# Critical-Infrastructure-Systems-Lab/ldsr

Hardware: AMD Instinct MI355X
Metric: restart x EM-iteration / s (T=1000, p=1, q=2) (higher is better)
Workload: dtype f64; 1 GPU; cfg2: synthetic T=1000 p=1 q=2, 1 series x 4096 restarts/GPU, niter=100, tol=0, dense mask; cells_rank0=4096, cells_total=4096, niter=100, algo=3

## Files before the change

ldsr_amd/csrc/em_pair_impl.h:

```cpp
#pragma once
#include "em_scan_impl.h"

__host__ __device__ constexpr long pair_image_doubles(int L, int PP, int QQ, int LPC = 32) {
    return img_doubles(L, LPC, PP, QQ);
}
__host__ __device__ constexpr long pair_strip_doubles(int L) { return (long)64 * (L - 1); }

__host__ __device__ constexpr long pair_tri_doubles(int PP, int QQ, int LPC = 32) {
    return (long)LPC * 2 * scan_pairs(PP, QQ);
}
#ifndef LDSR_STEADY
#define LDSR_STEADY 1
#endif
#ifndef LDSR_STEADY_PF
#define LDSR_STEADY_PF 4
#endif
#ifndef LDSR_STEADY_PF2
#define LDSR_STEADY_PF2 6
#endif
#ifndef LDSR_LEAD_CLOSED_VAR
#define LDSR_LEAD_CLOSED_VAR 1
#endif
#ifndef LDSR_STEADY_SBMASK
#define LDSR_STEADY_SBMASK 0x6
#endif
#ifndef LDSR_STEADY_MIN_L
#define LDSR_STEADY_MIN_L 24
#endif
#ifndef LDSR_PAIR_SPF
#define LDSR_PAIR_SPF 1
#endif
#ifndef LDSR_QUAD_SPF_LONG
#define LDSR_QUAD_SPF_LONG 1
#endif
#ifndef LDSR_PAIR_SPF_MAXL
#define LDSR_PAIR_SPF_MAXL 23
#endif
__host__ __device__ constexpr bool pair_spf(int PP, int QQ, int L, int LPC = 32) {
    return LDSR_PAIR_SPF && PP + QQ <= 8 && (L <= LDSR_PAIR_SPF_MAXL || (LDSR_QUAD_SPF_LONG && LPC == 16 && PP + QQ <= 4));
}
__host__ __device__ constexpr int pair_steady_ntr(int L, int LPC) { return L - 1; }
__host__ __device__ constexpr bool pair_steady(int L, int LPC, int PP, int QQ) {
    if (!LDSR_STEADY) return false;
    return LPC == 32 && L >= LDSR_STEADY_MIN_L &&
           (pair_image_doubles(L, PP, QQ, LPC) + 8 * pair_strip_doubles(L) + pair_tri_doubles(PP, QQ, LPC)) * 8 <= 160 * 1024;
}

__host__ __device__ constexpr bool pair_wide(int PP, int QQ) { return PP > 4 || QQ > 4; }
__host__ __device__ constexpr bool pair_member_fits(int L, int LPC, int PP, int QQ) {
    return (pair_image_doubles(L, PP, QQ, LPC) + (pair_wide(PP, QQ) ? 4 : 8) * pair_strip_doubles(L)) * 8 <= 160 * 1024;
}
constexpr int kPairLeadMaxL = 16;
__host__ __device__ constexpr bool pair_variant(int PP, int QQ, int L, int LPC, bool queue, bool lead) {
    if (!pair_member_fits(L, LPC, PP, QQ) || (lead && L > kPairLeadMaxL)) return false;
    return pair_wide(PP, QQ) ? lead && queue : true;
}

__device__ __forceinline__ double shfl_d(double x, int src_lane) { return __shfl(x, src_lane, 64); }

template <int LPC>
__device__ __forceinline__ void rscan_cross(double &P, double &G, double &H, int lane) {
    if constexpr (LPC == 32) {
        const double G1 = readlane_d(G, 16), H1 = readlane_d(H, 16), P1 = readlane_d(P, 16);
        const double G3 = readlane_d(G, 48), H3 = readlane_d(H, 48), P3 = readlane_d(P, 48);
        const int row = lane >> 4;
        const double Gs = row == 0 ? G1 : row == 2 ? G3 : 0.0;
        const double Hs = row == 0 ? H1 : row == 2 ? H3 : 0.0;
        const double Ps = row == 0 ? P1 : row == 2 ? P3 : 1.0;
        G = fma(P, Gs, G);
        H = fma(P * P, Hs, H);
        P *= Ps;
    }
}

#ifndef LDSR_LEAD_PIPE
#define LDSR_LEAD_PIPE 1
#endif
#ifndef LDSR_LEAD_PIPE_MAXP
#define LDSR_LEAD_PIPE_MAXP 2
#endif
__host__ __device__ constexpr bool lead_pipe(int PP) { return LDSR_LEAD_PIPE && PP <= LDSR_LEAD_PIPE_MAXP; }
template <int PP, int LPC, typename F>
__device__ __forceinline__ void lead_walk(const double *lup, int nj, int nA, F &&step) {
    constexpr int G = PP >= 4 ? 1 : 4 / PP;
    constexpr long ROW = (long)LPC * PP;
    double ua[G][PP], ub[G][PP];
    auto rd = [&](const double *base, double (&w)[G][PP]) {
#pragma unroll
        for (int i = 0; i < G; i++)
#pragma unroll
            for (int p_ = 0; p_ < PP; p_++) w[i][p_] = base[i * ROW + p_];
    };
    auto rdc = [&](int j0, double (&w)[G][PP]) {
#pragma unroll
        for (int i = 0; i < G; i++) {
            const int jj = min(j0 + i, nA - 1);
#pragma unroll
            for (int p_ = 0; p_ < PP; p_++) w[i][p_] = lup[jj * ROW + p_];
        }
    };
    if (nj <= 0) return;
    int j0 = 0;
    rdc(0, ua);
    const double *base = lup;
    for (; j0 + 3 * G <= nj; j0 += 2 * G, base += 2 * G * ROW) {
        rd(base + G * ROW, ub);
#pragma unroll
        for (int i = 0; i < G; i++) step(j0 + i, ua[i]);
        rd(base + 2 * G * ROW, ua);
#pragma unroll
        for (int i = 0; i < G; i++) step(j0 + G + i, ub[i]);
    }
    double uc[G][PP];
    rdc(j0 + G, ub);
    rdc(j0 + 2 * G, uc);
#pragma unroll
    for (int i = 0; i < G; i++)
        if (j0 + i < nj) step(j0 + i, ua[i]);
#pragma unroll
    for (int i = 0; i < G; i++)
        if (j0 + G + i < nj) step(j0 + G + i, ub[i]);
#pragma unroll
    for (int i = 0; i < G; i++)
        if (j0 + 2 * G + i < nj) step(j0 + 2 * G + i, uc[i]);
}

template <int PP, int QQ>
struct PairSweepOut {
    double aSyx, aTx1x, aPall, aSxx, likq, lsp, tLv, X0v, V0v;
    double aSxv[QQ], aTx1u[PP], aTux[PP];
    int sneg;
};

template <int PP, int QQ, int L, int LPC, bool DENSE>
__device__ __forceinline__ void pair_generic_sweeps(PairSweepOut<PP, QQ> &o, const Theta<PP, QQ> &th,
                                                    const double *ys, double *hs, unsigned obsmask,
                                                    int lane, int nl, int rp, double x_t1, double v_t1) {
    constexpr int KV = img_values(PP, QQ);
    const int vl = lane & (LPC - 1);
    auto val = [&](int j, int i) -> double { return ys[img_off(j, i, KV, LPC, L) + vl * 2]; };
    auto Yat = [&](int j) { return val(j, 0); };
    auto Uat = [&](int j, int k) { return val(j, 1 + k); };
    auto Vat = [&](int j, int k) { return val(j, 1 + PP + k); };
    constexpr bool SPF = pair_spf(PP, QQ, L, LPC) && (L <= LDSR_PAIR_SPF_MAXL || DENSE);
    constexpr int SPFD = scan_pairs(PP, QQ) <= 2 ? 2 : 1;
    constexpr int SPFN = SPFD + 1;
    constexpr int KH2 = 2 * (KV / 2);
    constexpr bool KODD = (KV & 1) != 0;
    struct StepRing {
        double w[SPFN][KH2 > 0 ? KH2 : 1];
        double o[2][2];
    };
    auto ring_rd = [&](double (&w)[KH2 > 0 ? KH2 : 1], double (&o)[2][2], int jn, bool with_odd) {
#pragma unroll
        for (int i = 0; i < KH2; i++) w[i] = val(jn, i);
        if (KODD && with_odd) {
            o[(jn >> 1) & 1][0] = val(jn & ~1, KV - 1);
            o[(jn >> 1) & 1][1] = val(jn | 1, KV - 1);
        }
    };
    const bool act = vl < nl, tail = vl < rp;
    const int lastLane = nl - 1;
    const double A = th.A, C = th.C, Q = th.Q, R = th.R;
    const double A2 = A * A, C2 = C * C;
    const double rR = fast_rcp(R);
    const double C2R = C2 * rR, ACR = A * C * rR, alpha = fma(Q, C2R, A2);
    auto e_at = [&](int j) {
        double e = Yat(j);
#pragma unroll
        for (int q_ = 0; q_ < QQ; q_++) e = fma(-th.D[q_], Vat(j, q_), e);
        return e;
    };
    auto bu_at = [&](int j) {
        double bu = 0.0;
#pragma unroll
        for (int p_ = 0; p_ < PP; p_++) bu = fma(th.B[p_], Uat(j, p_), bu);
        return bu;
    };
    auto e_of = [&](const double (&w)[KH2 > 0 ? KH2 : 1], const double (&o)[2][2], int j) {
        auto vv = [&](int i) { return i < KH2 ? w[i] : o[(j >> 1) & 1][j & 1]; };
        double e = vv(0);
#pragma unroll
        for (int q_ = 0; q_ < QQ; q_++) e = fma(-th.D[q_], vv(1 + PP + q_), e);
        return e;
    };
    auto bu_of = [&](const double (&w)[KH2 > 0 ? KH2 : 1], const double (&o)[2][2], int j) {
        auto vv = [&](int i) { return i < KH2 ? w[i] : o[(j >> 1) & 1][j & 1]; };
        double bu = 0.0;
#pragma unroll
        for (int p_ = 0; p_ < PP; p_++) bu = fma(th.B[p_], vv(1 + p_), bu);
        return bu;
    };
    double Jv[L], gv_[L];
    double hlast = 0.0;
    double likq = 0.0, lsp = 0.0, tLv = 0.0, X0v = 0.0, V0v = 0.0;
    int sneg = 0;
    double aSyx = 0.0, aTx1x = 0.0, aPall = 0.0, aSxx = 0.0;
    double aSxv[QQ], aTx1u[PP], aTux[PP];
#pragma unroll
    for (int q_ = 0; q_ < QQ; q_++) aSxv[q_] = 0.0;
#pragma unroll
    for (int p_ = 0; p_ < PP; p_++) { aTx1u[p_] = 0.0; aTux[p_] = 0.0; }

    PMat M;
    M.m00 = 1.0; M.m01 = 0.0; M.m10 = 0.0; M.m11 = 1.0; M.m20 = 0.0; M.m21 = 0.0; M.m22 = 1.0;
    if constexpr (DENSE) {
        const double mx = fmax(alpha, 1.0);
        const int ke = -__builtin_amdgcn_frexp_exp(mx);
        const double c = __builtin_amdgcn_ldexp(1.0, ke), cinv = __builtin_amdgcn_ldexp(1.0, -ke);
        const double al_ = alpha * c, Q_ = Q * c, C2R_ = C2R * c, A_ = A * c;
        double p00 = al_, p01 = Q_, p10 = C2R_, p11 = c;
        double q00 = 1.0, q01 = 0.0, q10 = 0.0, q11 = 1.0;
        bool have = false;
#pragma unroll
        for (int bit = 0; (1 << bit) <= L - 1; bit++) {
            if ((L - 1) & (1 << bit)) {
                if (!have) { q00 = p00; q01 = p01; q10 = p10; q11 = p11; have = true; }
                else {
                    const double t00 = fma(q00, p00, q01 * p10), t01 = fma(q00, p01, q01 * p11);
                    const double t10 = fma(q10, p00, q11 * p10), t11 = fma(q10, p01, q11 * p11);
// ... 23 lines not shown
                StepRing r;
#pragma unroll
                for (int d = 0; d < SPFD; d++)
                    if (L - 1 - d >= 0) ring_rd(r.w[(L - 1 - d) % SPFN], r.o, L - 1 - d, d == 0 || ((L - 1 - d) & 1) != 0);
                __builtin_amdgcn_sched_barrier(0x6);
#pragma unroll
                for (int j = L - 1; j >= 0; j--) {
                    if (j - SPFD >= 0) ring_rd(r.w[(j - SPFD) % SPFN], r.o, j - SPFD, ((j - SPFD) & 1) != 0);
                    if (j < L - 1 || tail) row_c(j, e_of(r.w[j % SPFN], r.o, j), bu_of(r.w[j % SPFN], r.o, j));
                    __builtin_amdgcn_sched_barrier(0x6);
                }
            } else {
                if (tail) row(L - 1);
#pragma unroll
                for (int j = L - 2; j >= 0; j--) row(j);
            }
            M.m00 = tail ? r00 : q00; M.m01 = tail ? r01 : q01;
            M.m10 = tail ? r10 : q10; M.m11 = tail ? r11 : q11;
            M.m20 = ra; M.m21 = rb; M.m22 = rcc * cinv;
            prenorm(M);
        }
    } else if (act) {
        auto f1c = [&](int j, double e, double bu) {
            const bool o = (obsmask >> j) & 1u;
            gv_[j] = e; Jv[j] = bu;
            const double a00 = o ? alpha : A2;
            const double g = o ? C2R : 0.0;
            const double s20 = o ? fma(bu, C2R, ACR * e) : 0.0;
            if (j == 0) {
                M.m00 = a00; M.m01 = Q; M.m10 = g; M.m11 = 1.0; M.m20 = s20; M.m21 = bu; M.m22 = A;
            } else {
                M = pstep(a00, Q, g, s20, bu, A, M);
            }
            if ((j & 15) == 15 && j < L - 2) prenorm(M);
        };
        auto f1 = [&](int j) { f1c(j, e_at(j), bu_at(j)); };
        if constexpr (SPF) {
            StepRing r;
#pragma unroll
            for (int d = 0; d < SPFD; d++)
                if (d <= L - 1) ring_rd(r.w[d % SPFN], r.o, d, (d & 1) == 0);
            __builtin_amdgcn_sched_barrier(0x6);
#pragma unroll
            for (int j = 0; j < L - 1; j++) {
                if (j + SPFD <= L - 1) ring_rd(r.w[(j + SPFD) % SPFN], r.o, j + SPFD, ((j + SPFD) & 1) == 0);
                f1c(j, e_of(r.w[j % SPFN], r.o, j), bu_of(r.w[j % SPFN], r.o, j));
                __builtin_amdgcn_sched_barrier(0x6);
            }
            if (tail) f1c(L - 1, e_of(r.w[(L - 1) % SPFN], r.o, L - 1), bu_of(r.w[(L - 1) % SPFN], r.o, L - 1));
        } else {
#pragma unroll
            for (int j = 0; j < L - 1; j++) f1(j);
            if (tail) f1(L - 1);
        }
        prenorm(M);
    }

    M = pmul(M, pdpp<DPP_ROW_SHR(1), 0xF>(M));
    M = pmul(M, pdpp<DPP_ROW_SHR(2), 0xF>(M));
    M = pmul(M, pdpp<DPP_ROW_SHR(4), 0xF>(M));
    prenorm(M);
    M = pmul(M, pdpp<DPP_ROW_SHR(8), 0xF>(M));
    if constexpr (LPC >= 32) M = pmul(M, pdpp<DPP_ROW_BCAST15, 0xA>(M));
    const double n_in = v_t1, d_in = 1.0, x_in = x_t1;
    double n_e = fma(M.m00, n_in, M.m01 * d_in);
    double d_e = fma(M.m10, n_in, M.m11 * d_in);
    double x_e = fma(M.m20, n_in, fma(M.m21, d_in, M.m22 * x_in));
    n_e = dppd<DPP_WAVE_SHR1, 0xF>(n_in, n_e);
    d_e = dppd<DPP_WAVE_SHR1, 0xF>(d_in, d_e);
    x_e = dppd<DPP_WAVE_SHR1, 0xF>(x_in, x_e);
    if (vl == 0) { n_e = n_in; d_e = d_in; x_e = x_in; }
    double Xp, Vp;
    {
        const double rd = fast_rcp(d_e);
        Vp = n_e * rd;
        Xp = x_e * rd;
    }

    double sprod = 1.0, Xu = 0.0, Vu = 0.0;
    int sexp = 0;
    double sg = fma(C2, Vp, R);
    double r0 = fast_rcp(sg);
    double Pi = 1.0, G = 0.0, H = 0.0;
    auto f2 = [&](int j) {
        const bool o = DENSE || ((obsmask >> j) & 1u);
        const double e = gv_[j], bu = Jv[j];
        const double r = o ? r0 : 0.0;
        const double sl = o ? sg : 1.0;
        sprod *= sl;
        sneg |= __double2hiint(sl);
        if ((j & 7) == 7) {
            sexp += __builtin_amdgcn_frexp_exp(sprod);
            sprod = __builtin_amdgcn_frexp_mant(sprod);
        }
        const double w = Vp * r;
        const double K = C * w;
        if (DENSE) Vu = R * w;
        else Vu = fma(-(C2 * w), Vp, Vp);
        const double dl = fma(-C, Xp, e);
        Xu = fma(K, dl, Xp);
        likq = fma(dl * r, dl, likq);
        const double Vp1 = fma(A2, Vu, Q);
        const double Xp1 = fma(A, Xu, bu);
        sg = fma(C2, Vp1, R);
        const double z = fast_rcp(sg * Vp1);
        const double rp1 = sg * z;
        r0 = Vp1 * z;
        const double AVu = A * Vu;
        double J = AVu * rp1;
        double g = fma(-J, Xp1, Xu);
        double h = fma(-J, AVu, Vu);
        if (j >= L - 2) {
            const bool fin = (vl == lastLane) && (j == (tail ? L - 1 : L - 2));
            J = fin ? 0.0 : J;
            g = fin ? Xu : g;
            h = fin ? Vu : h;
        }
        Jv[j] = J; gv_[j] = g;
        if (j < L - 1) hs[j * 64] = h; else hlast = h;
        G = fma(Pi, g, G);
        H = fma(Pi * Pi, h, H);
        Pi *= J;
        Xp = Xp1;
        Vp = Vp1;
        if ((j & 7) == 7) __builtin_amdgcn_sched_barrier(0);
    };
    if (act) {
#pragma unroll
        for (int j = 0; j < L - 1; j++) f2(j);
        if (tail) f2(L - 1);
    }
    tLv = fma(Xu, Xu, Vu);
    lsp = fma((double)sexp, 0.69314718055994530942, log_pos(sprod));

#define RSCAN_ROUND(n)                                                     \
    {                                                                  \
        const double Pb = dpp1<DPP_ROW_SHL(n)>(Pi);                    \
        const double Gb = dppz<DPP_ROW_SHL(n)>(G);                     \
        const double Hb = dppz<DPP_ROW_SHL(n)>(H);                     \
        G = fma(Pi, Gb, G);                                            \
        H = fma(Pi * Pi, Hb, H);                                       \
        Pi *= Pb;                                                      \
    }
    RSCAN_ROUND(1) RSCAN_ROUND(2) RSCAN_ROUND(4) RSCAN_ROUND(8)
#undef RSCAN_ROUND
    rscan_cross<LPC>(Pi, G, H, lane);
    double Xn = dppd<DPP_WAVE_SHL1, 0xF>(0.0, G);
    double Vn = dppd<DPP_WAVE_SHL1, 0xF>(0.0, H);
    if (vl == LPC - 1) { Xn = 0.0; Vn = 0.0; }

    const double XnE = Xn;
    auto b2a_h = [&](int j, double h) {
        const bool o = DENSE || ((obsmask >> j) & 1u);
        const double J = Jv[j];
        aTx1x = fma(Vn, J, aTx1x);
        const double Xs = fma(J, Xn, gv_[j]);
        const double Vs = fma(J * J, Vn, h);
        aPall += Vs;
        if (!DENSE) aSxx += o ? Vs : 0.0;
        gv_[j] = Xs;
        Xn = Xs;
        Vn = Vs;
    };
    auto b2a = [&](int j) { b2a_h(j, (j < L - 1) ? hs[j * 64] : hlast); };
    auto b2b_v = [&](int j, bool top, auto &&vv) {
        const bool o = DENSE || ((obsmask >> j) & 1u);
        const double Xs = gv_[j];
        const double Xnx = top ? XnE : gv_[top ? j : j + 1];
        aTx1x = fma(Xnx, Xs, aTx1x);
#pragma unroll
        for (int p_ = 0; p_ < PP; p_++) {
            const double ut = vv(1 + p_);
            aTx1u[p_] = fma(Xnx, ut, aTx1u[p_]);
            aTux[p_] = fma(ut, Xs, aTux[p_]);
        }
        aPall = fma(Xs, Xs, aPall);
        const double xo = o ? Xs : 0.0;
        aSyx = fma(vv(0), xo, aSyx);
        if (!DENSE) aSxx = fma(xo, xo, aSxx);
#pragma unroll
        for (int q_ = 0; q_ < QQ; q_++) aSxv[q_] = fma(xo, vv(1 + PP + q_), aSxv[q_]);
        if (!SPF && (j & 7) == 0) __builtin_amdgcn_sched_barrier(0);
    };
    auto b2b = [&](int j, bool top) { b2b_v(j, top, [&](int k) { return val(j, k); }); };
    if (act) {
        if constexpr (SPF) {
            StepRing r;
#pragma unroll
            for (int d = 0; d < SPFD; d++)
                if (L - 1 - d >= 0) ring_rd(r.w[(L - 1 - d) % SPFN], r.o, L - 1 - d, d == 0 || ((L - 1 - d) & 1) != 0);
            constexpr int HPF = 2;
            double hr[HPF + 1];
#pragma unroll
            for (int d = 0; d < HPF; d++)
                if (L - 2 - d >= 0) hr[(L - 2 - d) % (HPF + 1)] = hs[(L - 2 - d) * 64];
            __builtin_amdgcn_sched_barrier(0x6);
            if (tail) b2a_h(L - 1, hlast);
            else gv_[L - 1] = XnE;
#pragma unroll
            for (int j = L - 2; j >= 0; j--) {
                if (j - HPF >= 0) hr[(j - HPF) % (HPF + 1)] = hs[(j - HPF) * 64];
                b2a_h(j, hr[j % (HPF + 1)]);
                __builtin_amdgcn_sched_barrier(0x6);
            }
#pragma unroll
            for (int j = L - 1; j >= 0; j--) {
                if (j - SPFD >= 0) ring_rd(r.w[(j - SPFD) % SPFN], r.o, j - SPFD, ((j - SPFD) & 1) != 0);
                auto vv = [&](int k) { return k < KH2 ? r.w[j % SPFN][k] : r.o[(j >> 1) & 1][j & 1]; };
                if (j == L - 1) { if (tail) b2b_v(L - 1, true, vv); }
                else b2b_v(j, false, vv);
                __builtin_amdgcn_sched_barrier(0x6);
            }
        } else {
            if (tail) b2a(L - 1);
            else gv_[L - 1] = XnE;
#pragma unroll
// ... 400 lines not shown
#ifdef LDSR_SCAN_TIMING
    unsigned long long tick_[10], last_, real0_;
#endif
};
#ifdef LDSR_SCAN_TIMING
#define PAIR_TICK_REFS auto &tick_ = cs.tick_; auto &last_ = cs.last_;
#else
#define PAIR_TICK_REFS
#endif

__device__ __forceinline__ int pair_cell_at(const PairEnv &E, int c0, int pos) { return E.perm ? E.perm[c0 + pos] : c0 + pos; }

__device__ __forceinline__ void pair_mark_interrupted(const PairEnv &E, int cell) {
    const int P = 6 + E.p + E.q;
    for (int k = 0; k < P; k++) E.theta[(long)cell * P + k] = NAN;
    if (E.liks && E.liks_nanfill)
        for (int i = 0; i < E.niter; i++) E.liks[(long)cell * E.niter + i] = NAN;
    E.n_iter[cell] = 0;
    E.lik[cell] = NAN;
    E.status[cell] = 3;
}

struct PairVarBlk { double Vp, sg, r0, K, Vu, AVu, J, Vp1; bool st; };
template <int L>
__device__ __forceinline__ PairVarBlk pair_var_block(double V1, double A, double C, double Q, double R, bool live,
                                                     int vl, int hbase, bool shape_ok) {
    constexpr int LPC = 32, NTR = L - 1;
    PairVarBlk b;
    const double A2 = A * A, C2 = C * C;
    const double C2R = C2 * fast_rcp(R), alpha = fma(Q, C2R, A2);
    const bool trl = vl < NTR;
    double Vp;
    {
        const double mxs = fmax(alpha, 1.0);
        const int ke = -__builtin_amdgcn_frexp_exp(mxs);
        const double cs = __builtin_amdgcn_ldexp(1.0, ke);
        double p00 = trl ? alpha * cs : 1.0, p01 = trl ? Q * cs : 0.0;
        double p10 = trl ? C2R * cs : 0.0, p11 = trl ? cs : 1.0;
#define VSCAN_ROUND(Q00, Q01, Q10, Q11)                                                      \
        {                                                                            \
            const double q00 = Q00, q01 = Q01, q10 = Q10, q11 = Q11;                 \
            const double r00 = fma(p00, q00, p01 * q10), r01 = fma(p00, q01, p01 * q11); \
            const double r10 = fma(p10, q00, p11 * q10), r11 = fma(p10, q01, p11 * q11); \
            p00 = r00; p01 = r01; p10 = r10; p11 = r11;                              \
        }
#define VSCAN_SHR(n) VSCAN_ROUND(dpp1<DPP_ROW_SHR(n)>(p00), dppz<DPP_ROW_SHR(n)>(p01), dppz<DPP_ROW_SHR(n)>(p10), dpp1<DPP_ROW_SHR(n)>(p11))
        VSCAN_SHR(1) VSCAN_SHR(2) VSCAN_SHR(4)
        {
            const double m = fmax(fmax(fabs(p00), fabs(p01)), fmax(fabs(p10), fabs(p11)));
            const int e2 = 1 - __builtin_amdgcn_frexp_exp(m);
            p00 = __builtin_amdgcn_ldexp(p00, e2); p01 = __builtin_amdgcn_ldexp(p01, e2);
            p10 = __builtin_amdgcn_ldexp(p10, e2); p11 = __builtin_amdgcn_ldexp(p11, e2);
        }
        VSCAN_SHR(8)
        VSCAN_ROUND((dppd<DPP_ROW_BCAST15, 0xA>(1.0, p00)), (dppd<DPP_ROW_BCAST15, 0xA>(0.0, p01)),
                    (dppd<DPP_ROW_BCAST15, 0xA>(0.0, p10)), (dppd<DPP_ROW_BCAST15, 0xA>(1.0, p11)))
#undef VSCAN_SHR
#undef VSCAN_ROUND
        double n_e = fma(p00, V1, p01), d_e = fma(p10, V1, p11);
        n_e = dppd<DPP_WAVE_SHR1, 0xF>(V1, n_e);
        d_e = dppd<DPP_WAVE_SHR1, 0xF>(1.0, d_e);
        if (vl == 0) { n_e = V1; d_e = 1.0; }
        Vp = n_e * fast_rcp(d_e);
    }
    const double sg = fma(C2, Vp, R);
    const double r0 = fast_rcp(sg);
    const double w = Vp * r0;
    b.K = C * w;
    b.Vu = R * w;
    b.Vp1 = fma(A2, b.Vu, Q);
    b.AVu = A * b.Vu;
    b.J = b.AVu * fast_rcp(b.Vp1);
    b.Vp = Vp; b.sg = sg; b.r0 = r0;
    const double dV = b.Vp1 - Vp;
    const bool conv = fabs(dV) <= 3.552713678800501e-15 * fabs(Vp) && Vp > 0.0 && b.J * b.J < 0.8;
    const unsigned long long okm = __ballot(sg > 0.0 && sg < INFINITY);
    const unsigned long long cvm = __ballot(conv);
    constexpr unsigned long long CELL = (1ull << LPC) - 1ull;
    const unsigned long long hm = (okm >> hbase) & CELL, hc = (cvm >> hbase) & CELL;
    b.st = live && hm == CELL && ((hc >> (LPC - 1)) & 1ull) != 0ull && shape_ok;
    return b;
}

template <int PP, int QQ, bool QUEUE>
__device__ __forceinline__ void pair_steady_finish(const PairEnv &E, PairCarry<PP, QQ> &cs, const PairSweepOut<PP, QQ> &o,
                                                   double addTx1x, double addPall, bool active, int lane, int c0,
                                                   int nc, int lastLane) {
    constexpr int LPC = 32;
    PAIR_TICK_REFS
    const int vl = lane & 31, hbase = lane & 32;
    const int P = 6 + E.p + E.q;
    Sums<PP, QQ> S;
    {
        constexpr int NB = 5;
        constexpr int NR = NB + QQ + 2 * PP;
        double red[NR];
        red[0] = o.aSyx; red[1] = o.aTx1x; red[2] = o.aPall; red[3] = o.likq; red[4] = o.lsp;
#pragma unroll
        for (int q_ = 0; q_ < QQ; q_++) red[NB + q_] = o.aSxv[q_];
#pragma unroll
        for (int p_ = 0; p_ < PP; p_++) { red[NB + QQ + p_] = o.aTx1u[p_]; red[NB + QQ + PP + p_] = o.aTux[p_]; }
        red_rounds<NR, LPC / 2>(red, lane);
        {
            const double tt = red[0];
#pragma unroll
            for (int i = 0; i < NR; i++) red[i] = shfl_d(tt, hbase | red_home(i, NR, LPC));
        }
        S.X0 = shfl_d(o.X0v, hbase);
        S.V0 = shfl_d(o.V0v, hbase);
        const double termLast = shfl_d(o.tLv, hbase | lastLane);
        red[1] += addTx1x; red[2] += addPall;
        const double term0 = fma(S.X0, S.X0, S.V0);
        const unsigned long long negm = __ballot(o.sneg < 0);
        const bool neg = ((negm >> hbase) & ((1ull << LPC) - 1ull)) != 0;
        S.Syx = red[0]; S.Tx1x = red[1];
        S.Sxx = red[2];
#pragma unroll
        for (int q_ = 0; q_ < QQ; q_++) S.Sxv[q_] = red[NB + q_];
#pragma unroll
        for (int p_ = 0; p_ < PP; p_++) { S.Tx1u[p_] = red[NB + QQ + p_]; S.Tux[p_] = red[NB + QQ + PP + p_]; }
        S.Txx = red[2] - termLast;
        S.Tx1x1 = red[2] - term0;
        if (active) {
            cs.lik2 = cs.lik1;
            cs.lik1 = cs.lik;
            cs.lik = (-0.5 * E.n_obs * LDSR_LOG_2PI - 0.5 * (red[3] + red[4])) / E.n_obs;
            if (neg) cs.lik = NAN;
        }
    }
    SCAN_TICK(8)
    int abort_now = 0;
    if (E.abort && ((++cs.wit) & 63) == 0)
        abort_now = __builtin_amdgcn_readfirstlane(lane == 0 ? ldsr_poll_abort(E.abort) : 0);
    if (active && E.liks && vl == 0) E.liks[(long)cs.cell * E.niter + cs.it] = cs.lik;
    if (active) cs.it++;
    bool stop = active && cs.it >= E.niter;
    if (active && cs.it >= 3 && fabs(cs.lik - cs.lik1) < E.tol && fabs(cs.lik1 - cs.lik2) < E.tol) stop = true;
    if (cs.alive && abort_now) stop = true;
    if (cs.alive && stop) {
        white_out(cs.th, (SeriesConstK)E.sc);
        if (vl == 0) {
            store_theta(cs.th, E.theta + (long)cs.cell * P, E.p, E.q);
            if (E.liks && E.liks_nanfill)
                for (int i = cs.it; i < E.niter; i++) E.liks[(long)cs.cell * E.niter + i] = NAN;
            E.n_iter[cs.cell] = cs.it;
            E.lik[cs.cell] = cs.lik;
            E.status[cs.cell] = (abort_now && cs.it < E.niter) ? 3 : (isfinite(cs.lik) ? 0 : 1);
#ifdef LDSR_SCAN_TIMING
            tick_[9] = __builtin_amdgcn_s_memrealtime() - cs.real0_;
            if (E.liks && E.niter >= 10)
                for (int k_ = 0; k_ < 10; k_++) E.liks[(long)cs.cell * E.niter + k_] = (double)tick_[k_];
#endif
        }
        cs.alive = false;
        if constexpr (QUEUE) {
            if (abort_now) {
                for (int pulls = 0; pulls <= nc; pulls++) {
                    int kn = 0;
                    if (vl == 0) kn = atomicAdd(E.queue_s, 1);
                    kn = __shfl(kn, hbase, 64);
                    if (kn >= nc) break;
                    if (vl == 0) pair_mark_interrupted(E, pair_cell_at(E, c0, kn));
                }
            } else {
                int kn = 0;
                if (vl == 0) kn = atomicAdd(E.queue_s, 1);
                kn = __shfl(kn, hbase, 64);
                if (kn < nc) {
                    cs.alive = true;
                    cs.cell = pair_cell_at(E, c0, kn);
                    load_theta(cs.th, E.theta0 + (long)cs.cell * P, E.p, E.q, E.has_u, E.has_v);
                    white_in(cs.th, (SeriesConstK)E.sc);
                    cs.it = 0;
                    cs.lik = NAN; cs.lik1 = NAN; cs.lik2 = NAN;
                }
            }
        }
    } else if (active) {
        mstep_update_white<PP, QQ>(cs.th, S, (SeriesConstK)E.sc, E.T);
    }
}

template <int PP, int QQ, int L, bool QUEUE>
__device__ __attribute__((noinline)) PairCarry<PP, QQ> pair_steady_g_phase(PairEnv Ev, PairCarry<PP, QQ> cs, bool slow,
                                                                           int c0, int nc) {
    constexpr int LPC = 32;
    extern __shared__ __attribute__((aligned(16))) double smem[];
    PAIR_TICK_REFS
    auto ui = [](int x) { return __builtin_amdgcn_readfirstlane(x); };
    auto up = [&](auto *ptr) {
        const unsigned long long v = (unsigned long long)ptr;
        const unsigned lo = (unsigned)__builtin_amdgcn_readfirstlane((int)(unsigned)v);
        const unsigned hi = (unsigned)__builtin_amdgcn_readfirstlane((int)(unsigned)(v >> 32));
        return (decltype(ptr))(((unsigned long long)hi << 32) | lo);
    };
    PairEnv E;
    E.T = ui(Ev.T); E.p = ui(Ev.p); E.q = ui(Ev.q); E.has_u = ui(Ev.has_u); E.has_v = ui(Ev.has_v);
    E.niter = ui(Ev.niter); E.liks_nanfill = ui(Ev.liks_nanfill); E.n_obs = ui(Ev.n_obs);
    E.tol = uniform_d(Ev.tol);
    E.sc = up(Ev.sc); E.queue_s = up(Ev.queue_s); E.perm = up(Ev.perm); E.theta0 = up(Ev.theta0);
    E.theta = up(Ev.theta); E.lik = up(Ev.lik); E.liks = up(Ev.liks); E.n_iter = up(Ev.n_iter);
    E.status = up(Ev.status); E.abort = up(Ev.abort);
    c0 = ui(c0); nc = ui(nc);
    const int lane = threadIdx.x & 63, wave = threadIdx.x >> 6;
    const int vl = lane & 31, hbase = lane & 32;
    const int T = E.T;
    const int nl = (T + L - 1) / L, rp = T - nl * (L - 1);
    const bool shape_ok = rp >= 1 && nl > 1;
    const double *ys = smem;
    double *hs = smem + pair_image_doubles(L, PP, QQ, LPC) + (long)wave * pair_strip_doubles(L) + lane;
    do {
        SCAN_TICK(7)
        PairSweepOut<PP, QQ> o;
        pair_generic_sweeps<PP, QQ, L, LPC, true>(o, cs.th, ys, hs, 0u, lane, nl, rp, cs.th.mu1, cs.th.V1);
        SCAN_TICK(6)
        pair_steady_finish<PP, QQ, QUEUE>(E, cs, o, 0.0, 0.0, slow, lane, c0, nc, nl - 1);
        const PairVarBlk vb = pair_var_block<L>(cs.th.V1, cs.th.A, cs.th.C, cs.th.Q, cs.th.R, cs.alive, vl, hbase, shape_ok);
        slow = cs.alive && !vb.st;
    } while (__any(slow));
    return cs;
}

template <int PP, int QQ, int L, bool QUEUE>
__device__ __forceinline__ void em_pair_body_steady(const EmParams &prm, const double *ys, double *hs,
                                                    const double *tri, int s, int c0, int nc, int lane,
                                                    int wave) {
    constexpr int LPC = 32;
    constexpr int KP = scan_pairs(PP, QQ), KV = img_values(PP, QQ);
    constexpr int NTR = L - 1;
    static_assert(NTR < LPC, "the last lane of the cell is the template, not a transient step");
    const int vl = lane & 31, hbase = lane & 32;
    auto val = [&](int j, int i) -> double { return ys[img_off(j, i, KV, LPC, L) + vl * 2]; };
    auto ldw = [&](int j, double (&w)[2 * KP]) {
#pragma unroll
        for (int i = 0; i < KV; i++) w[i] = val(j, i);
    };
    constexpr int PF = KP <= 2 ? LDSR_STEADY_PF : (KP <= 4 ? 2 : 1);
    constexpr int PF2 = LDSR_STEADY_PF2;
    const int T = prm.T;
    const int P = 6 + prm.p + prm.q;
    PairEnv E;
    E.T = T; E.p = prm.p; E.q = prm.q; E.has_u = prm.has_u; E.has_v = prm.has_v;
    E.niter = prm.niter; E.liks_nanfill = prm.liks_nanfill; E.tol = prm.tol;
    E.sc = prm.sc + s; E.n_obs = E.sc->n_obs;
    E.queue_s = prm.queue + s; E.perm = prm.perm; E.theta0 = prm.theta0;
    E.theta = prm.theta; E.lik = prm.lik; E.liks = prm.liks; E.n_iter = prm.n_iter; E.status = prm.status;
    E.abort = prm.abort;
    const int nl = (T + L - 1) / L;
    const int rp = T - nl * (L - 1);
    const bool act = vl < nl;
    const bool tail = vl < rp;
    const int lastLane = nl - 1;
    const bool shape_ok = rp >= 1 && nl > 1;

    PairCarry<PP, QQ> cs;
    int k = QUEUE ? 0 : 2 * wave + (lane >> 5);
    if constexpr (QUEUE) {
        if (vl == 0) k = atomicAdd(E.queue_s, 1);
        k = __shfl(k, hbase, 64);
    }
    cs.alive = k < nc;
    cs.cell = pair_cell_at(E, c0, cs.alive ? k : 0);
    load_theta(cs.th, prm.theta0 + (long)cs.cell * P, prm.p, prm.q, prm.has_u, prm.has_v);
    white_in(cs.th, (SeriesConstK)E.sc);
    cs.lik = NAN; cs.lik1 = NAN; cs.lik2 = NAN;
    cs.it = 0;
    cs.wit = 0;
#ifdef LDSR_SCAN_TIMING
    for (int k_ = 0; k_ < 10; k_++) cs.tick_[k_] = 0;
    cs.last_ = __builtin_readcyclecounter();
    cs.real0_ = __builtin_amdgcn_s_memrealtime();
#endif
    PAIR_TICK_REFS
    Theta<PP, QQ> &th = cs.th;

    while (__any(cs.alive)) {
        bool slow = false;
        while (__any(cs.alive)) {
            SCAN_TICK(7)
            const double A = th.A, C = th.C;
            const PairVarBlk vb = pair_var_block<L>(th.V1, A, C, th.Q, th.R, cs.alive, vl, hbase, shape_ok);
            const bool st = vb.st;
            slow = cs.alive && !st;
            if (__builtin_expect(__any(slow), 0)) break;
            double likq = 0.0, lsp = 0.0, tLv = 0.0, X0v = 0.0, V0v = 0.0;
            double addPall = 0.0, addTx1x = 0.0;
            double aSyx = 0.0, aTx1x = 0.0, aPall = 0.0;
            double aSxv[QQ], aTx1u[PP], aTux[PP];
            auto zero_sums = [&]() {
                aSyx = 0.0; aTx1x = 0.0; aPall = 0.0;
#pragma unroll
                for (int q_ = 0; q_ < QQ; q_++) aSxv[q_] = 0.0;
#pragma unroll
                for (int p_ = 0; p_ < PP; p_++) { aTx1u[p_] = 0.0; aTux[p_] = 0.0; }
            };
            const bool trl = vl < NTR;
            auto tval = [&](int i) -> double { return tri[((i >> 1) * LPC + vl) * 2 + (i & 1)]; };
            double e_t = tval(0), bu_t = 0.0;
#pragma unroll
            for (int q_ = 0; q_ < QQ; q_++) e_t = fma(-th.D[q_], tval(1 + PP + q_), e_t);
#pragma unroll
            for (int p_ = 0; p_ < PP; p_++) bu_t = fma(th.B[p_], tval(1 + p_), bu_t);
            const double K = vb.K, J = vb.J, Vu = vb.Vu, AVu = vb.AVu, r0 = vb.r0;
            double Xp;
            {
                const double aKt = A * K;
                double al = trl ? fma(-aKt, C, A) : 1.0, bl = trl ? fma(aKt, e_t, bu_t) : 0.0;
#define MSCAN_ROUND(AB, BB) { const double ab = AB, bb = BB; bl = fma(al, bb, bl); al *= ab; }
                MSCAN_ROUND(dpp1<DPP_ROW_SHR(1)>(al), dppz<DPP_ROW_SHR(1)>(bl))
                MSCAN_ROUND(dpp1<DPP_ROW_SHR(2)>(al), dppz<DPP_ROW_SHR(2)>(bl))
                MSCAN_ROUND(dpp1<DPP_ROW_SHR(4)>(al), dppz<DPP_ROW_SHR(4)>(bl))
                MSCAN_ROUND(dpp1<DPP_ROW_SHR(8)>(al), dppz<DPP_ROW_SHR(8)>(bl))
                MSCAN_ROUND((dppd<DPP_ROW_BCAST15, 0xA>(1.0, al)), (dppd<DPP_ROW_BCAST15, 0xA>(0.0, bl)))
#undef MSCAN_ROUND
                Xp = fma(al, th.mu1, bl);
                Xp = dppd<DPP_WAVE_SHR1, 0xF>(th.mu1, Xp);
                if (vl == 0) Xp = th.mu1;
            }
            const double dl = fma(-C, Xp, e_t);
            const double Xu = fma(K, dl, Xp);
            const double Xp1 = fma(A, Xu, bu_t);
            const double trJ = J;
            const double trG = fma(-J, Xp1, Xu);
            const double trH = fma(-J, AVu, Vu);
            const double trLq = trl ? dl * r0 * dl : 0.0;
            const double lg = log_pos(vb.sg);
            const double trLg = trl ? lg : 0.0;
            const int src = hbase | (LPC - 1);
            const double cK = shfl_d(K, src), cJ = shfl_d(J, src), cr = shfl_d(r0, src), cVu = shfl_d(Vu, src);
            const double ch = shfl_d(trH, src), clg = shfl_d(lg, src), X_tr = shfl_d(Xp, src);

            SCAN_TICK(0)
            if (st) {
                const bool body = act && vl >= 1;
                const bool tail_s = tail;
                const double aK = A * cK, a = fma(-aK, C, A);
                double aL = 1.0, JL = 1.0;
                {
                    double sa = a, sj = cJ;
                    bool have = false;
#pragma unroll
                    for (int bit = 0; (1 << bit) <= L - 1; bit++) {
                        if ((L - 1) & (1 << bit)) {
                            if (!have) { aL = sa; JL = sj; have = true; }
                            else { aL *= sa; JL *= sj; }
                        }
                        if ((2 << bit) <= L - 1) { sa *= sa; sj *= sj; }
                    }
                }
                double gv_[L];
                double al = 1.0, bl = 0.0, buLast = 0.0;
                auto f1s = [&](int j, const double (&w)[2 * KP]) {
                    double e = w[0], bu = 0.0;
#pragma unroll
                    for (int q_ = 0; q_ < QQ; q_++) e = fma(-th.D[q_], w[1 + PP + q_], e);
#pragma unroll
                    for (int p_ = 0; p_ < PP; p_++) bu = fma(th.B[p_], w[1 + p_], bu);
                    gv_[j] = e;
                    if (j < L - 1) hs[j * 64] = bu; else buLast = bu;
                    bl = fma(a, bl, fma(aK, e, bu));
                };
                {
                    constexpr bool PRET = KP <= 4;
                    double Wt[2 * KP], W[PF][2 * KP];
                    if constexpr (PRET) ldw(L - 1, Wt);
#pragma unroll
                    for (int d = 0; d < PF; d++) ldw(d, W[d]);
                    __builtin_amdgcn_sched_barrier(LDSR_STEADY_SBMASK);
                    if (body) {
#pragma unroll
                        for (int j = 0; j < L - 1; j++) {
                            f1s(j, W[j % PF]);
                            if (j + PF < L - 1) ldw(j + PF, W[j % PF]);
                            __builtin_amdgcn_sched_barrier(LDSR_STEADY_SBMASK);
                        }
                        al = aL;
                    }
                    if (tail_s) {
                        if constexpr (!PRET) ldw(L - 1, Wt);
                        f1s(L - 1, Wt);
                        al *= a;
                    }
                }
#define SSCAN_ROUND(AB, BB) { const double ab = AB, bb = BB; bl = fma(al, bb, bl); al *= ab; }
                SSCAN_ROUND(dpp1<DPP_ROW_SHR(1)>(al), dppz<DPP_ROW_SHR(1)>(bl))
                SSCAN_ROUND(dpp1<DPP_ROW_SHR(2)>(al), dppz<DPP_ROW_SHR(2)>(bl))
                SSCAN_ROUND(dpp1<DPP_ROW_SHR(4)>(al), dppz<DPP_ROW_SHR(4)>(bl))
                SSCAN_ROUND(dpp1<DPP_ROW_SHR(8)>(al), dppz<DPP_ROW_SHR(8)>(bl))
                SSCAN_ROUND((dppd<DPP_ROW_BCAST15, 0xA>(1.0, al)), (dppd<DPP_ROW_BCAST15, 0xA>(0.0, bl)))
#undef SSCAN_ROUND
                SCAN_TICK(1)
                double Xq = fma(al, X_tr, bl);
                Xq = dppd<DPP_WAVE_SHR1, 0xF>(X_tr, Xq);
                if (vl == 0) Xq = X_tr;
                double lq = 0.0, Xuq = 0.0;
                auto f2s = [&](int j, double bu) {
                    const double e = gv_[j];
                    const double dlq = fma(-C, Xq, e);
                    lq = fma(dlq, dlq, lq);
                    Xuq = fma(cK, dlq, Xq);
                    const double Xq1 = fma(A, Xuq, bu);
                    double g = fma(-cJ, Xq1, Xuq);
                    if (j >= L - 2) {
                        const bool fin = (vl == lastLane) && (j == (tail_s ? L - 1 : L - 2));
                        g = fin ? Xuq : g;
                    }
                    gv_[j] = g;
                    Xq = Xq1;
                };
                if (body) {
                    double U[PF2];
#pragma unroll
                    for (int d = 0; d < PF2; d++) U[d] = hs[d * 64];
                    __builtin_amdgcn_sched_barrier(LDSR_STEADY_SBMASK);
#pragma unroll
                    for (int j = 0; j < L - 1; j++) {
                        f2s(j, U[j % PF2]);
                        if (j + PF2 < L - 1) U[j % PF2] = hs[(j + PF2) * 64];
                        __builtin_amdgcn_sched_barrier(LDSR_STEADY_SBMASK);
                    }
                }
                if (tail_s) f2s(L - 1, buLast);
                SCAN_TICK(2)
                constexpr bool PRET2 = KP <= 4;
                double Vt[2 * KP], V[PF][2 * KP];
                if constexpr (PRET2) {
                    ldw(L - 1, Vt);
#pragma unroll
                    for (int d = 0; d < PF; d++) ldw(L - 2 - d, V[d]);
                }
                __builtin_amdgcn_sched_barrier(LDSR_STEADY_SBMASK);
                tLv = fma(Xuq, Xuq, cVu);
                const int nst = (body ? L - 1 : 0) + (tail_s ? 1 : 0);
                likq = fma(cr, lq, trLq);
                lsp = fma((double)nst, clg, trLg);
                double Pi = 1.0, G = 0.0;
                if (tail_s) { G = gv_[L - 1]; Pi = cJ; }
                if (body) {
#pragma unroll
                    for (int j = L - 2; j >= 0; j--) G = fma(cJ, G, gv_[j]);
                    Pi *= JL;
                }
#define RSCAN_ROUND(n) { const double Pb = dpp1<DPP_ROW_SHL(n)>(Pi), Gb = dppz<DPP_ROW_SHL(n)>(G); G = fma(Pi, Gb, G); Pi *= Pb; }
                RSCAN_ROUND(1) RSCAN_ROUND(2) RSCAN_ROUND(4) RSCAN_ROUND(8)
#undef RSCAN_ROUND
                {
                    double Hdummy = 0.0;
                    rscan_cross<LPC>(Pi, G, Hdummy, lane);
                }
                double Xn = dppd<DPP_WAVE_SHL1, 0xF>(0.0, G);
                if (vl == LPC - 1) Xn = 0.0;
                const double XsS = shfl_d(G, hbase);
                SCAN_TICK(3)
                zero_sums();
                auto b2s = [&](int j, const double (&w)[2 * KP]) {
                    const double Xs = fma(cJ, Xn, gv_[j]);
                    aTx1x = fma(Xn, Xs, aTx1x);
#pragma unroll
                    for (int p_ = 0; p_ < PP; p_++) {
                        const double ut = w[1 + p_];
                        aTx1u[p_] = fma(Xn, ut, aTx1u[p_]);
                        aTux[p_] = fma(ut, Xs, aTux[p_]);
                    }
                    aPall = fma(Xs, Xs, aPall);
                    aSyx = fma(w[0], Xs, aSyx);
#pragma unroll
                    for (int q_ = 0; q_ < QQ; q_++) aSxv[q_] = fma(Xs, w[1 + PP + q_], aSxv[q_]);
                    Xn = Xs;
                };
                if constexpr (!PRET2) {
                    if (tail_s) ldw(L - 1, Vt);
#pragma unroll
                    for (int d = 0; d < PF; d++) ldw(L - 2 - d, V[d]);
                }
                if (tail_s) b2s(L - 1, Vt);
                if (body) {
#pragma unroll
                    for (int j = L - 2; j >= 0; j--) {
                        const int d = (L - 2 - j) % PF;
                        b2s(j, V[d]);
                        if (j - PF >= 0) ldw(j - PF, V[d]);
                        __builtin_amdgcn_sched_barrier(LDSR_STEADY_SBMASK);
                    }
                }
                SCAN_TICK(4)
                const int N = T - NTR;
                const double rho = cJ * cJ;
                const double romr = fast_rcp(1.0 - rho);
                const double Vss = ch * romr;
                const double dV = cVu - Vss;
                const double VsS = Vss;
                const double sumVs = fma(dV, romr, (double)N * Vss);
                addPall = sumVs;
                addTx1x = cJ * (sumVs - VsS);
                {
                    int vl2 = vl;
                    asm volatile("" : "+v"(vl2));
                    auto tval2 = [&](int i) -> double { return tri[((i >> 1) * LPC + vl2) * 2 + (i & 1)]; };
                    double Pt = trl ? trJ : 1.0, Gt = trl ? trG : 0.0, Ht = trl ? trH : 0.0;
#define RSCAN_ROUND(n)                                                     \
                    {                                                          \
                        const double Pb = dpp1<DPP_ROW_SHL(n)>(Pt);            \
                        const double Gb = dppz<DPP_ROW_SHL(n)>(Gt);            \
                        const double Hb = dppz<DPP_ROW_SHL(n)>(Ht);            \
                        Gt = fma(Pt, Gb, Gt);                                  \
                        Ht = fma(Pt * Pt, Hb, Ht);                             \
                        Pt *= Pb;                                              \
                    }
                    RSCAN_ROUND(1) RSCAN_ROUND(2) RSCAN_ROUND(4) RSCAN_ROUND(8)
#undef RSCAN_ROUND
                    rscan_cross<LPC>(Pt, Gt, Ht, lane);
                    const double XsT = fma(Pt, XsS, Gt), VsT = fma(Pt * Pt, VsS, Ht);
                    const double XsN = dppd<DPP_WAVE_SHL1, 0xF>(0.0, XsT);
                    const double VsN = dppd<DPP_WAVE_SHL1, 0xF>(0.0, VsT);
                    if (trl) {
                        aTx1x = fma(XsN, XsT, fma(VsN, trJ, aTx1x));
#pragma unroll
                        for (int p_ = 0; p_ < PP; p_++) {
                            const double ut = tval2(1 + p_);
                            aTx1u[p_] = fma(XsN, ut, aTx1u[p_]);
                            aTux[p_] = fma(ut, XsT, aTux[p_]);
                        }
                        aPall += fma(XsT, XsT, VsT);
                        aSyx = fma(tval2(0), XsT, aSyx);
#pragma unroll
                        for (int q_ = 0; q_ < QQ; q_++) aSxv[q_] = fma(XsT, tval2(1 + PP + q_), aSxv[q_]);
                    }
                    X0v = XsT; V0v = VsT;
                }
            } else {
                zero_sums();
            }
            SCAN_TICK(5)
            PairSweepOut<PP, QQ> o;
            o.aSyx = aSyx; o.aTx1x = aTx1x; o.aPall = aPall; o.aSxx = 0.0;
            o.likq = likq; o.lsp = lsp; o.tLv = tLv; o.X0v = X0v; o.V0v = V0v; o.sneg = 0;
#pragma unroll
            for (int q_ = 0; q_ < QQ; q_++) o.aSxv[q_] = aSxv[q_];
#pragma unroll
            for (int p_ = 0; p_ < PP; p_++) { o.aTx1u[p_] = aTx1u[p_]; o.aTux[p_] = aTux[p_]; }
            pair_steady_finish<PP, QQ, QUEUE>(E, cs, o, addTx1x, addPall, st, lane, c0, nc, lastLane);
        }
        if (__builtin_expect(!__any(slow), 1)) break;
        cs = pair_steady_g_phase<PP, QQ, L, QUEUE>(E, cs, slow, c0, nc);
    }
}

template <int PP, int QQ, int L, int LPC, bool QUEUE, bool LEAD = false>
__global__ __launch_bounds__(512) void em_pair_kernel(EmParams prm) {
    extern __shared__ __attribute__((aligned(16))) double smem[];
    constexpr long IMG = pair_image_doubles(L, PP, QQ, LPC);
    const int b = blockIdx.x;
    const int s = prm.blk_series[b];
    const int c0 = prm.blk_cell0[b], nc = prm.blk_ncell[b];
    const int lane = threadIdx.x & 63, wave = threadIdx.x >> 6;
    const double *gimg = prm.img2 + (long)s * prm.img2_stride;
    for (int i = threadIdx.x; i < (int)IMG; i += blockDim.x) smem[i] = gimg[i];
    constexpr long STRIP = pair_strip_doubles(L);
    double *lu = smem + IMG + (long)(blockDim.x >> 6) * STRIP;
    if constexpr (LEAD) {
        const int n3 = ((prm.lead + LPC - 1) / LPC) * LPC * PP;
        const double *g3 = prm.img3 + (long)s * prm.img3_stride;
        for (int i = threadIdx.x; i < n3; i += blockDim.x) lu[i] = g3[i];
    }
    constexpr bool STEADY = !LEAD && pair_steady(L, LPC, PP, QQ);
    const double *tri = lu;
    if constexpr (STEADY) {
        constexpr int KP = scan_pairs(PP, QQ);
        constexpr int NTR = pair_steady_ntr(L, LPC);
        for (int i = threadIdx.x; i < KP * LPC * 2; i += blockDim.x) {
            const int c = i & 1, l = (i >> 1) % LPC, m = (i >> 1) / LPC;
            const int vi = 2 * m + c;
            lu[i] = (l < NTR && vi < img_values(PP, QQ)) ? gimg[img_off(l % L, vi, img_values(PP, QQ), LPC, L) + (l / L) * 2] : 0.0;
        }
    }
    __syncthreads();
    const SeriesConst *sc = prm.sc + s;
    if (sc->status != 0) {
        const int P = 6 + prm.p + prm.q;
        for (int c = threadIdx.x; c < nc; c += blockDim.x) {
            const int cell = c0 + c;
            for (int k = 0; k < P; k++) prm.theta[(long)cell * P + k] = NAN;
            prm.n_iter[cell] = 0;
            if (prm.liks && prm.liks_nanfill)
                for (int i = 0; i < prm.niter; i++) prm.liks[(long)cell * prm.niter + i] = NAN;
            prm.lik[cell] = NAN;
            prm.status[cell] = 2;
        }
        return;
    }
    if (!QUEUE && (64 / LPC) * wave >= nc) return;
    double *hs = smem + IMG + (long)wave * STRIP + lane;
    const bool dense = sc->n_obs == prm.T;
    if constexpr (LEAD) {
        em_pair_body<PP, QQ, L, LPC, false, QUEUE, true>(prm, smem, hs, lu, s, c0, nc, lane, wave);
    } else {
        if (dense) {
            if constexpr (STEADY) em_pair_body_steady<PP, QQ, L, QUEUE>(prm, smem, hs, tri, s, c0, nc, lane, wave);
            else em_pair_body<PP, QQ, L, LPC, true, QUEUE, false>(prm, smem, hs, lu, s, c0, nc, lane, wave);
        } else {
            em_pair_body<PP, QQ, L, LPC, false, QUEUE, false>(prm, smem, hs, lu, s, c0, nc, lane, wave);
        }
    }
}

struct PairPlan {
    int L = 0;
    int lpc = 0;
    int wpb = 0;
    bool ok = false;
};
PairPlan pair_plan(int T, int PP, int QQ, int lpc, bool lead_form = false);

template <int L, int LPC>
hipError_t launch_em_pair_L(const EmParams &prm, int PPv, int QQv, int n_blocks, int wpb, bool queue,
                            hipStream_t stream);
__host__ __device__ constexpr long pair_lead_doubles(int lead, int LPC, int PP) {
    return (long)((lead + LPC - 1) / LPC) * LPC * PP;
}
```

Before: 557.1 million restart*EM-iter/s.

## Compute log-likelihood only on iterations that need it

```diff
diff --git a/ldsr_amd/csrc/em_pair_impl.h b/ldsr_amd/csrc/em_pair_impl.h
--- a/ldsr_amd/csrc/em_pair_impl.h
+++ b/ldsr_amd/csrc/em_pair_impl.h
@@ -1,4 +1,5 @@
 #pragma once
+#include <type_traits>
 #include "em_scan_impl.h"
 
 __host__ __device__ constexpr long pair_image_doubles(int L, int PP, int QQ, int LPC = 32) {
@@ -26,6 +27,9 @@
 #endif
 #ifndef LDSR_STEADY_MIN_L
 #define LDSR_STEADY_MIN_L 24
+#endif
+#ifndef LDSR_LIK_ON_DEMAND
+#define LDSR_LIK_ON_DEMAND 1
 #endif
 #ifndef LDSR_PAIR_SPF
 #define LDSR_PAIR_SPF 1
@@ -132,10 +136,12 @@
     int sneg;
 };
 
-template <int PP, int QQ, int L, int LPC, bool DENSE>
+template <int PP, int QQ, int L, int LPC, bool DENSE, bool LIKOD = false>
 __device__ __forceinline__ void pair_generic_sweeps(PairSweepOut<PP, QQ> &o, const Theta<PP, QQ> &th,
                                                     const double *ys, double *hs, unsigned obsmask,
-                                                    int lane, int nl, int rp, double x_t1, double v_t1) {
+                                                    int lane, int nl, int rp, double x_t1, double v_t1,
+                                                    bool need_lik = true) {
+    static_assert(!LIKOD || DENSE, "likelihood on demand: fully observed series only");
     constexpr int KV = img_values(PP, QQ);
     const int vl = lane & (LPC - 1);
     auto val = [&](int j, int i) -> double { return ys[img_off(j, i, KV, LPC, L) + vl * 2]; };
@@ -325,16 +331,48 @@
     double sg = fma(C2, Vp, R);
     double r0 = fast_rcp(sg);
     double Pi = 1.0, G = 0.0, H = 0.0;
+    if constexpr (LIKOD) {
+        if (need_lik) {
+            if (act) {
+                double Xl = Xp, Vl = Vp, sgl = sg, rl = r0;
+                auto f2l = [&](int j) {
+                    const double e = gv_[j], bu = Jv[j];
+                    sprod *= sgl;
+                    sneg |= __double2hiint(sgl);
+                    if ((j & 7) == 7) {
+                        sexp += __builtin_amdgcn_frexp_exp(sprod);
+                        sprod = __builtin_amdgcn_frexp_mant(sprod);
+                    }
+                    const double w = Vl * rl;
+                    const double K = C * w;
+                    const double Vul = R * w;
+                    const double dl = fma(-C, Xl, e);
+                    const double Xul = fma(K, dl, Xl);
+                    likq = fma(dl * rl, dl, likq);
+                    Vl = fma(A2, Vul, Q);
+                    Xl = fma(A, Xul, bu);
+                    sgl = fma(C2, Vl, R);
+                    rl = Vl * fast_rcp(sgl * Vl);
+                };
+#pragma unroll
+                for (int j = 0; j < L - 1; j++) f2l(j);
+                if (tail) f2l(L - 1);
+            }
+            lsp = fma((double)sexp, 0.69314718055994530942, log_pos(sprod));
+        }
+    }
     auto f2 = [&](int j) {
         const bool o = DENSE || ((obsmask >> j) & 1u);
         const double e = gv_[j], bu = Jv[j];
         const double r = o ? r0 : 0.0;
-        const double sl = o ? sg : 1.0;
-        sprod *= sl;
-        sneg |= __double2hiint(sl);
-        if ((j & 7) == 7) {
-            sexp += __builtin_amdgcn_frexp_exp(sprod);
-            sprod = __builtin_amdgcn_frexp_mant(sprod);
+        if constexpr (!LIKOD) {
+            const double sl = o ? sg : 1.0;
+            sprod *= sl;
+            sneg |= __double2hiint(sl);
+            if ((j & 7) == 7) {
+                sexp += __builtin_amdgcn_frexp_exp(sprod);
+                sprod = __builtin_amdgcn_frexp_mant(sprod);
+            }
         }
         const double w = Vp * r;
         const double K = C * w;
@@ -342,7 +380,7 @@
         else Vu = fma(-(C2 * w), Vp, Vp);
         const double dl = fma(-C, Xp, e);
         Xu = fma(K, dl, Xp);
-        likq = fma(dl * r, dl, likq);
+        if constexpr (!LIKOD) likq = fma(dl * r, dl, likq);
         const double Vp1 = fma(A2, Vu, Q);
         const double Xp1 = fma(A, Xu, bu);
         sg = fma(C2, Vp1, R);
@@ -374,7 +412,7 @@
         if (tail) f2(L - 1);
     }
     tLv = fma(Xu, Xu, Vu);
-    lsp = fma((double)sexp, 0.69314718055994530942, log_pos(sprod));
+    if constexpr (!LIKOD) lsp = fma((double)sexp, 0.69314718055994530942, log_pos(sprod));
 
 #define RSCAN_ROUND(n)                                                     \
     {                                                                  \
@@ -941,51 +979,68 @@
     return b;
 }
 
+template <int PP, int QQ, bool WL>
+__device__ __forceinline__ void pair_steady_reduce(const PairEnv &E, PairCarry<PP, QQ> &cs, const PairSweepOut<PP, QQ> &o,
+                                                   Sums<PP, QQ> &S, double addTx1x, double addPall, bool active,
+                                                   int lane, int lastLane) {
+    constexpr int LPC = 32;
+    const int hbase = lane & 32;
+    constexpr int NB = WL ? 5 : 3;
+    constexpr int NR = NB + QQ + 2 * PP;
+    double red[NR];
+    red[0] = o.aSyx; red[1] = o.aTx1x; red[2] = o.aPall;
+    if constexpr (WL) { red[3] = o.likq; red[4] = o.lsp; }
+#pragma unroll
+    for (int q_ = 0; q_ < QQ; q_++) red[NB + q_] = o.aSxv[q_];
+#pragma unroll
+    for (int p_ = 0; p_ < PP; p_++) { red[NB + QQ + p_] = o.aTx1u[p_]; red[NB + QQ + PP + p_] = o.aTux[p_]; }
+    red_rounds<NR, LPC / 2>(red, lane);
+    {
+        const double tt = red[0];
+#pragma unroll
+        for (int i = 0; i < NR; i++) red[i] = shfl_d(tt, hbase | red_home(i, NR, LPC));
+    }
+    S.X0 = shfl_d(o.X0v, hbase);
+    S.V0 = shfl_d(o.V0v, hbase);
+    const double termLast = shfl_d(o.tLv, hbase | lastLane);
+    red[1] += addTx1x; red[2] += addPall;
+    const double term0 = fma(S.X0, S.X0, S.V0);
+    const unsigned long long negm = WL ? __ballot(o.sneg < 0) : 0ull;
+    const bool neg = ((negm >> hbase) & ((1ull << LPC) - 1ull)) != 0;
+    S.Syx = red[0]; S.Tx1x = red[1];
+    S.Sxx = red[2];
+#pragma unroll
+    for (int q_ = 0; q_ < QQ; q_++) S.Sxv[q_] = red[NB + q_];
+#pragma unroll
+    for (int p_ = 0; p_ < PP; p_++) { S.Tx1u[p_] = red[NB + QQ + p_]; S.Tux[p_] = red[NB + QQ + PP + p_]; }
+    S.Txx = red[2] - termLast;
+    S.Tx1x1 = red[2] - term0;
+    if constexpr (WL) {
+        if (active) {
+            cs.lik2 = cs.lik1;
+            cs.lik1 = cs.lik;
+            cs.lik = (-0.5 * E.n_obs * LDSR_LOG_2PI - 0.5 * (red[3] + red[4])) / E.n_obs;
+            if (neg) cs.lik = NAN;
+        }
+    } else {
+        if (active) cs.lik = NAN;
+    }
+}
+
 template <int PP, int QQ, bool QUEUE>
 __device__ __forceinline__ void pair_steady_finish(const PairEnv &E, PairCarry<PP, QQ> &cs, const PairSweepOut<PP, QQ> &o,
                                                    double addTx1x, double addPall, bool active, int lane, int c0,
-                                                   int nc, int lastLane) {
+                                                   int nc, int lastLane, bool need_lik) {
     constexpr int LPC = 32;
     PAIR_TICK_REFS
     const int vl = lane & 31, hbase = lane & 32;
     const int P = 6 + E.p + E.q;
     Sums<PP, QQ> S;
-    {
-        constexpr int NB = 5;
-        constexpr int NR = NB + QQ + 2 * PP;
-        double red[NR];
-        red[0] = o.aSyx; red[1] = o.aTx1x; red[2] = o.aPall; red[3] = o.likq; red[4] = o.lsp;
-#pragma unroll
-        for (int q_ = 0; q_ < QQ; q_++) red[NB + q_] = o.aSxv[q_];
-#pragma unroll
-        for (int p_ = 0; p_ < PP; p_++) { red[NB + QQ + p_] = o.aTx1u[p_]; red[NB + QQ + PP + p_] = o.aTux[p_]; }
-        red_rounds<NR, LPC / 2>(red, lane);
-        {
-            const double tt = red[0];
-#pragma unroll
-            for (int i = 0; i < NR; i++) red[i] = shfl_d(tt, hbase | red_home(i, NR, LPC));
-        }
-        S.X0 = shfl_d(o.X0v, hbase);
-        S.V0 = shfl_d(o.V0v, hbase);
-        const double termLast = shfl_d(o.tLv, hbase | lastLane);
-        red[1] += addTx1x; red[2] += addPall;
-        const double term0 = fma(S.X0, S.X0, S.V0);
-        const unsigned long long negm = __ballot(o.sneg < 0);
-        const bool neg = ((negm >> hbase) & ((1ull << LPC) - 1ull)) != 0;
-        S.Syx = red[0]; S.Tx1x = red[1];
-        S.Sxx = red[2];
-#pragma unroll
-        for (int q_ = 0; q_ < QQ; q_++) S.Sxv[q_] = red[NB + q_];
-#pragma unroll
-        for (int p_ = 0; p_ < PP; p_++) { S.Tx1u[p_] = red[NB + QQ + p_]; S.Tux[p_] = red[NB + QQ + PP + p_]; }
-        S.Txx = red[2] - termLast;
-        S.Tx1x1 = red[2] - term0;
-        if (active) {
-            cs.lik2 = cs.lik1;
-            cs.lik1 = cs.lik;
-            cs.lik = (-0.5 * E.n_obs * LDSR_LOG_2PI - 0.5 * (red[3] + red[4])) / E.n_obs;
-            if (neg) cs.lik = NAN;
-        }
+    if constexpr (QUEUE) {
+        pair_steady_reduce<PP, QQ, true>(E, cs, o, S, addTx1x, addPall, active, lane, lastLane);
+    } else {
+        if (need_lik) pair_steady_reduce<PP, QQ, true>(E, cs, o, S, addTx1x, addPall, active, lane, lastLane);
+        else pair_steady_reduce<PP, QQ, false>(E, cs, o, S, addTx1x, addPall, active, lane, lastLane);
     }
     SCAN_TICK(8)
     int abort_now = 0;
@@ -1038,6 +1093,14 @@
     } else if (active) {
         mstep_update_white<PP, QQ>(cs.th, S, (SeriesConstK)E.sc, E.T);
     }
+}
+
+template <int PP, int QQ, bool QUEUE>
+__device__ __forceinline__ bool pair_need_lik(const PairEnv &E, const PairCarry<PP, QQ> &cs, bool active) {
+    if constexpr (QUEUE || LDSR_LIK_ON_DEMAND == 0) return true;
+    else if constexpr (LDSR_LIK_ON_DEMAND == 2) return false;
+    else return __any(E.tol > 0.0 || E.liks != nullptr || (active && cs.it + 1 >= E.niter) ||
+                      (E.abort != nullptr && ((cs.wit + 1) & 63) == 0)) != 0;
 }
 
 template <int PP, int QQ, int L, bool QUEUE>
@@ -1070,10 +1133,11 @@
     double *hs = smem + pair_image_doubles(L, PP, QQ, LPC) + (long)wave * pair_strip_doubles(L) + lane;
     do {
         SCAN_TICK(7)
+        const bool need_lik = pair_need_lik<PP, QQ, QUEUE>(E, cs, slow);
         PairSweepOut<PP, QQ> o;
-        pair_generic_sweeps<PP, QQ, L, LPC, true>(o, cs.th, ys, hs, 0u, lane, nl, rp, cs.th.mu1, cs.th.V1);
+        pair_generic_sweeps<PP, QQ, L, LPC, true, !QUEUE>(o, cs.th, ys, hs, 0u, lane, nl, rp, cs.th.mu1, cs.th.V1, need_lik);
         SCAN_TICK(6)
-        pair_steady_finish<PP, QQ, QUEUE>(E, cs, o, 0.0, 0.0, slow, lane, c0, nc, nl - 1);
+        pair_steady_finish<PP, QQ, QUEUE>(E, cs, o, 0.0, 0.0, slow, lane, c0, nc, nl - 1, need_lik);
         const PairVarBlk vb = pair_var_block<L>(cs.th.V1, cs.th.A, cs.th.C, cs.th.Q, cs.th.R, cs.alive, vl, hbase, shape_ok);
         slow = cs.alive && !vb.st;
     } while (__any(slow));
@@ -1142,6 +1206,7 @@
             const bool st = vb.st;
             slow = cs.alive && !st;
             if (__builtin_expect(__any(slow), 0)) break;
+            const bool need_lik = pair_need_lik<PP, QQ, QUEUE>(E, cs, cs.alive);
             double likq = 0.0, lsp = 0.0, tLv = 0.0, X0v = 0.0, V0v = 0.0;
             double addPall = 0.0, addTx1x = 0.0;
             double aSyx = 0.0, aTx1x = 0.0, aPall = 0.0;
@@ -1182,12 +1247,15 @@
             const double trJ = J;
             const double trG = fma(-J, Xp1, Xu);
             const double trH = fma(-J, AVu, Vu);
-            const double trLq = trl ? dl * r0 * dl : 0.0;
-            const double lg = log_pos(vb.sg);
-            const double trLg = trl ? lg : 0.0;
+            double trLq = 0.0, lg = 0.0, trLg = 0.0;
+            if (need_lik) {
+                trLq = trl ? dl * r0 * dl : 0.0;
+                lg = log_pos(vb.sg);
+                trLg = trl ? lg : 0.0;
+            }
             const int src = hbase | (LPC - 1);
             const double cK = shfl_d(K, src), cJ = shfl_d(J, src), cr = shfl_d(r0, src), cVu = shfl_d(Vu, src);
-            const double ch = shfl_d(trH, src), clg = shfl_d(lg, src), X_tr = shfl_d(Xp, src);
+            const double ch = shfl_d(trH, src), clg = need_lik ? shfl_d(lg, src) : 0.0, X_tr = shfl_d(Xp, src);
 
             SCAN_TICK(0)
             if (st) {
@@ -1253,10 +1321,26 @@
                 Xq = dppd<DPP_WAVE_SHR1, 0xF>(X_tr, Xq);
                 if (vl == 0) Xq = X_tr;
                 double lq = 0.0, Xuq = 0.0;
+                constexpr bool LOD = !QUEUE;
+                if constexpr (LOD) {
+                    if (need_lik) {
+                        double Xl = Xq;
+                        auto f2l = [&](int j, double bu) {
+                            const double dlq = fma(-C, Xl, gv_[j]);
+                            lq = fma(dlq, dlq, lq);
+                            Xl = fma(A, fma(cK, dlq, Xl), bu);
+                        };
+                        if (body) {
+#pragma unroll
+                            for (int j = 0; j < L - 1; j++) f2l(j, hs[j * 64]);
+                        }
+                        if (tail_s) f2l(L - 1, buLast);
+                    }
+                }
                 auto f2s = [&](int j, double bu) {
                     const double e = gv_[j];
                     const double dlq = fma(-C, Xq, e);
-                    lq = fma(dlq, dlq, lq);
+                    if constexpr (!LOD) lq = fma(dlq, dlq, lq);
                     Xuq = fma(cK, dlq, Xq);
                     const double Xq1 = fma(A, Xuq, bu);
                     double g = fma(-cJ, Xq1, Xuq);
@@ -1291,8 +1375,10 @@
                 __builtin_amdgcn_sched_barrier(LDSR_STEADY_SBMASK);
                 tLv = fma(Xuq, Xuq, cVu);
                 const int nst = (body ? L - 1 : 0) + (tail_s ? 1 : 0);
-                likq = fma(cr, lq, trLq);
-                lsp = fma((double)nst, clg, trLg);
+                if (need_lik) {
+                    likq = fma(cr, lq, trLq);
+                    lsp = fma((double)nst, clg, trLg);
+                }
                 double Pi = 1.0, G = 0.0;
                 if (tail_s) { G = gv_[L - 1]; Pi = cJ; }
                 if (body) {
@@ -1398,7 +1484,7 @@
             for (int q_ = 0; q_ < QQ; q_++) o.aSxv[q_] = aSxv[q_];
 #pragma unroll
             for (int p_ = 0; p_ < PP; p_++) { o.aTx1u[p_] = aTx1u[p_]; o.aTux[p_] = aTux[p_]; }
-            pair_steady_finish<PP, QQ, QUEUE>(E, cs, o, addTx1x, addPall, st, lane, c0, nc, lastLane);
+            pair_steady_finish<PP, QQ, QUEUE>(E, cs, o, addTx1x, addPall, st, lane, c0, nc, lastLane, need_lik);
         }
         if (__builtin_expect(!__any(slow), 1)) break;
         cs = pair_steady_g_phase<PP, QQ, L, QUEUE>(E, cs, slow, c0, nc);
```

Measured after the change: 592.6 million restart*EM-iter/s (median of 6 runs). 6.4% higher.
